# emolch/kiwi

Hardware: AMD Instinct MI355X
Metric: trial-source misfit evals/s (higher is better)
Workload: dtype f32

## Files before the change

kiwi_amd/csrc/kiwi_accum.hip:

```cpp
#include "kiwi_accum_api.hpp"

#if KIWI_ARITH == 0
#define KIWI_ARITH_NS exact
#elif KIWI_ARITH == 1
#define KIWI_ARITH_NS fused
#else
#error "KIWI_ARITH: 0 (exact) or 1 (fused)"
#endif

namespace kiwi {
namespace KIWI_ARITH_NS {

#include "kiwi_accum.inc"

#define KIWI_COMMON_ARGS a.G, a.span, a.pitch, a.recs, a.cent_ofs, a.isrc0, a.nrec, a.recv, a.syn, a.syn_stride

#if KIWI_FAMILY == 1
void launch_direct(const AccumArgs &a, dim3 grid)
{
    if (a.ng == 10) hipLaunchKernelGGL(accumulate_kernel<10>, grid, dim3(256), 0, a.stream, KIWI_COMMON_ARGS, a.synrow);
    else            hipLaunchKernelGGL(accumulate_kernel<8>, grid, dim3(256), 0, a.stream, KIWI_COMMON_ARGS, a.synrow);
}
#endif

// ... 22 lines not shown
    } else {
        if (T == 64) grouped_t<8, 64>(a, grid, ntiles, runs, pairsel, mate, mate4);
        else if (T == 128) grouped_t<8, 128>(a, grid, ntiles, runs, pairsel, mate, mate4);
        else grouped_t<8, 256>(a, grid, ntiles, runs, pairsel, mate, mate4);
    }
}
#endif

#if KIWI_FAMILY == 3
template <int NG, int NS, bool COMPACT, bool PLAN>
static void multi_t(const AccumArgs &a, dim3 grid, int ntiles, const int *mate, const int *wider)
{
    if (a.fuse) hipLaunchKernelGGL((accumulate_multi_kernel<NG, true, NS, COMPACT, PLAN>), grid, dim3(256), 0, a.stream, KIWI_COMMON_ARGS, ntiles, a.tab, a.coefs, a.fp,
                                   a.pairflag, mate, wider, a.plan, a.plan_ofs);
    else        hipLaunchKernelGGL((accumulate_multi_kernel<NG, false, NS, COMPACT, PLAN>), grid, dim3(256), 0, a.stream, KIWI_COMMON_ARGS, ntiles, a.tab, a.coefs, a.fp,
                                   a.pairflag, mate, wider, a.plan, a.plan_ofs);
}
template <int NG, int NS>
static void multi_c(const AccumArgs &a, dim3 grid, int ntiles, const int *mate, const int *wider)
{
    if (a.compact && a.plan) multi_t<NG, NS, true, true>(a, grid, ntiles, mate, wider);
    else if (a.compact) multi_t<NG, NS, true, false>(a, grid, ntiles, mate, wider);
    else multi_t<NG, NS, false, false>(a, grid, ntiles, mate, wider);
}
void launch_multi(const AccumArgs &a, dim3 grid, int NS, int ntiles, const int *mate, const int *wider)
{
    if (a.ng == 10) { if (NS == 4) multi_c<10, 4>(a, grid, ntiles, mate, wider); else multi_c<10, 2>(a, grid, ntiles, mate, wider); }
    else            { if (NS == 4) multi_c<8, 4>(a, grid, ntiles, mate, wider); else multi_c<8, 2>(a, grid, ntiles, mate, wider); }
}
void launch_multi_plan(const AccumArgs &a, int NS, int ngroups, const int *mate, const int *wider, PlanSrc *plan)
{
    const dim3 grid((unsigned)ngroups, (unsigned)((a.nrec + 63) / 64));
    if (NS == 4) hipLaunchKernelGGL(multi_plan_kernel<4>, grid, dim3(64), 0, a.stream, a.recs, a.cent_ofs, a.isrc0, a.nrec, a.recv, a.tab, a.pairflag, mate, wider,
                                    a.plan_ofs, (int4 *)plan, a.plan_regular, a.plan_count);
    else         hipLaunchKernelGGL(multi_plan_kernel<2>, grid, dim3(64), 0, a.stream, a.recs, a.cent_ofs, a.isrc0, a.nrec, a.recv, a.tab, a.pairflag, mate, wider,
                                    a.plan_ofs, (int4 *)plan, a.plan_regular, a.plan_count);
}
#endif

#if KIWI_FAMILY == 4
template <int NG, bool COMPACT>
static void cell_t(const AccumArgs &a, dim3 grid, int ntiles, bool per_wave)
{
#define KIWI_C(KERNEL) hipLaunchKernelGGL(KERNEL, grid, dim3(256), 0, a.stream, KIWI_COMMON_ARGS, ntiles, a.tab, a.coefs, a.fp, a.pairflag, a.synrow, \
                                          a.fam_ofs, a.fam_list)
    if (per_wave) { if (a.fuse) KIWI_C((accumulate_cellw_kernel<NG, true, COMPACT>)); else KIWI_C((accumulate_cellw_kernel<NG, false, COMPACT>)); }
    else          { if (a.fuse) KIWI_C((accumulate_cell_kernel<NG, 256, 2, 0, true, COMPACT>)); else KIWI_C((accumulate_cell_kernel<NG, 256, 2, 0, false, COMPACT>)); }
#undef KIWI_C
}
template <int NG>
static void cell_c(const AccumArgs &a, dim3 grid, int ntiles, bool per_wave)
{
    if (a.compact) cell_t<NG, true>(a, grid, ntiles, per_wave); else cell_t<NG, false>(a, grid, ntiles, per_wave);
}
void launch_cell(const AccumArgs &a, dim3 grid, int ntiles) { if (a.ng == 10) cell_c<10>(a, grid, ntiles, false); else cell_c<8>(a, grid, ntiles, false); }
void launch_cellw(const AccumArgs &a, dim3 grid, int ntiles) { if (a.ng == 10) cell_c<10>(a, grid, ntiles, true); else cell_c<8>(a, grid, ntiles, true); }
int cellw_range() { return kCellwRange; }
#endif

}
}
```

kiwi_amd/csrc/kiwi_accum.inc:

```


typedef float f4u __attribute__((ext_vector_type(4), aligned(4)));
typedef float f2u __attribute__((ext_vector_type(2), aligned(4)));

#if defined(KIWI_EXPLICIT_FMA)
#ifndef KIWI_CELLW_AHEAD
#define KIWI_CELLW_AHEAD 3
#endif
template <class V> __device__ __forceinline__ V kiwi_mad(V acc, float w, V v)
{
    V ws;
    for (int k = 0; k < (int)(sizeof(V) / sizeof(float)); k++) ws[k] = w;
    return __builtin_elementwise_fma(ws, v, acc);
}
template <class V> __device__ __forceinline__ V kiwi_madv(V acc, V w, V v) { return __builtin_elementwise_fma(w, v, acc); }
#else
template <class V> __device__ __forceinline__ V kiwi_mad(V acc, float w, V v) { return acc + w * v; }
template <class V> __device__ __forceinline__ V kiwi_madv(V acc, V w, V v) { return acc + w * v; }
#endif

typedef int v4i_t __attribute__((ext_vector_type(4)));
typedef int v2i_t __attribute__((ext_vector_type(2)));
__device__ __forceinline__ __amdgpu_buffer_rsrc_t gf_rsrc(const float *base)
{
// ... 788 lines not shown
        if constexpr (i < nH1) {
            t1[0] = t1[0] + c1 * s2a<i>(H); t1[0] = t1[0] + c2 * s2a<i>(L);
            t1[1] = t1[1] + c1 * s2b<i>(H); t1[1] = t1[1] + c2 * s2b<i>(L);
        } else if constexpr (i < nH1 + 2) {
            t2[0] = t2[0] + c1 * s2a<i>(H); t2[0] = t2[0] + c2 * s2a<i>(L);
            t2[1] = t2[1] + c1 * s2b<i>(H); t2[1] = t2[1] + c2 * s2b<i>(L);
        } else {
            dz[0] = dz[0] + c1 * s2a<i>(H); dz[0] = dz[0] + c2 * s2a<i>(L);
            dz[1] = dz[1] + c1 * s2b<i>(H); dz[1] = dz[1] + c2 * s2b<i>(L);
        }
        if constexpr (i == nH1 + 1) {
#pragma unroll
            for (int k = 0; k < 2; k++) {
                if (ROT) {
                    ar1[k] = ar1[k] + cl * t1[k] - sl * t2[k];
                    ar2[k] = ar2[k] + cl * t2[k] + sl * t1[k];
                } else {
                    ar1[k] = t1[k]; ar2[k] = t2[k];
                }
            }
        }
    });
}

template <int NG>
__device__ __forceinline__ typename Set2Sel<NG>::type make_set2(f2v &a0, f2v &a1, f2v &a2, f2v &a3, f2v &a4, f2v &a5, f2v &a6, f2v &a7, f2v &a8, f2v &a9,
                                                                f2v &b0, f2v &b1, f2v &b2, f2v &b3, f2v &b4, f2v &b5, f2v &b6, f2v &b7, f2v &b8, f2v &b9)
{
    if constexpr (NG == 10) return Set2_10{ a0, a1, a2, a3, a4, a5, a6, a7, a8, a9, b0, b1, b2, b3, b4, b5, b6, b7, b8, b9 };
    else return Set2_8{ a0, a1, a2, a3, a4, a5, a6, a7, b0, b1, b2, b3, b4, b5, b6, b7 };
}

#include "kiwi_apply_asm.inc"
#include "kiwi_apply_plan_asm.inc"
__device__ __forceinline__ int coef_warm(const float *p)
{
    int d;
    asm volatile("s_load_dword %0, %1, 0x0\n\ts_load_dword %0, %1, 0x40\n\ts_load_dword %0, %1, 0x80\n\ts_load_dword %0, %1, 0xc0\n\t"
                 "s_load_dword %0, %1, 0x100\n\ts_load_dword %0, %1, 0x140\n\ts_load_dword %0, %1, 0x180\n\ts_load_dword %0, %1, 0x1c0"
                 : "=&s"(d) : "s"(p) : "memory");
    return d;
}
#if KIWI_ARITH == 1
#define KIWI_APPLY_ASM(NGV, KV, RV) apply_group_asm_##NGV##_k##KV##_##RV##_fused
#define KIWI_APPLY_PLAN(NGV, KV, RV) apply_plan_asm_##NGV##_k##KV##_##RV##_fused
#else
#define KIWI_APPLY_ASM(NGV, KV, RV) apply_group_asm_##NGV##_k##KV##_##RV##_exact
#define KIWI_APPLY_PLAN(NGV, KV, RV) apply_plan_asm_##NGV##_k##KV##_##RV##_exact
#endif

template <int NG, int T, bool FUSE, bool RUNS, bool COMPACT >
__global__ __launch_bounds__(T) __attribute__((amdgpu_waves_per_eu(3))) void accumulate_grouped_kernel(
    const float *__restrict__ G, const int2 *__restrict__ span, int pitch,
    const GeoRec *__restrict__ recs, const int *__restrict__ cent_ofs, int isrc0, int nrec,
    const RecvDev *__restrict__ recv, float *__restrict__ syn, size_t syn_stride, int ntiles,
    const int *__restrict__ tab, const float *__restrict__ coefs, const int *__restrict__ run_first, FuseParams fp,
    const int *__restrict__ pairflag ,
    int pairsel ,
    const int *__restrict__ mate, const int *__restrict__ mate4 ,
    const int *__restrict__ synrow ,
    const int *__restrict__ fam_ofs, const int *__restrict__ fam_list )
{
    constexpr bool compact = COMPACT;
    constexpr int TILE = 4 * T;
    constexpr int LDS_TILE = TILE + kHalo;
    __shared__ __attribute__((aligned(16))) float tiles[NG][LDS_TILE];
    const int s = RUNS ? run_first[blockIdx.x] : (int)blockIdx.x;
    const int s_end = RUNS ? run_first[blockIdx.x + 1] : s + 1;
    const bool multi = RUNS && s_end - s > 1;
    const int tile = blockIdx.y % ntiles, r = blockIdx.y / ntiles;
    const RecvDev &rv = recv[r];
    if (!rv.enabled) return;
    if (tile * TILE >= rv.wlen) return;
    if (pairsel == 1 && cell_pair(rv, pairflag, s, nrec, r)) return;
    if (pairsel == 3 && (multi_taken_fwd<4>(rv, pairflag, mate4, s, nrec, r) || multi_taken_fwd<2>(rv, pairflag, mate, s, nrec, r))) return;
    if (synrow && !multi && synrow[s] != s) return;
    const int tid = threadIdx.x;
    const int lane = tid & 63;
    const int t_tile0 = rv.wbeg + tile * TILE;
    const int cb = cent_ofs[isrc0], c0 = cent_ofs[isrc0 + s], nc = cent_ofs[isrc0 + s + 1] - c0;
    const GeoRec *__restrict__ rc = recs + ((size_t)(c0 - cb) * nrec + (size_t)r * nc);
// ... 457 lines not shown
            for (int s = 0; s < NS; s++)
                if (only < 0 || only == s) one_finish<true>(v[i], tile0 + s * SET, LDS_TILE, comp(i), p, gw[s]);
        }
        if (i + DEPTH < N && (i + DEPTH < N - 1 || last_ok)) issue(i + DEPTH);
    }
    if (whalo) {
#pragma unroll
        for (int s = 0; s < NS; s++)
            if (only < 0 || only == s) halo_finish<true>(hact, hv, tile0 + s * SET, LDS_TILE, hig, hph, gw[s]);
    }
}


__device__ __forceinline__ int smax_u(int a, int b) { int r; asm("s_max_i32 %0, %1, %2" : "=s"(r) : "s"(a), "s"(b) : "scc"); return r; }
__device__ __forceinline__ int smin_u(int a, int b) { int r; asm("s_min_i32 %0, %1, %2" : "=s"(r) : "s"(a), "s"(b) : "scc"); return r; }

template <int NS>
__device__ __forceinline__ bool multi_taken(const RecvDev &rv, const int *__restrict__ pairflag, const int *__restrict__ mate,
                                            int s, int nrec, int r)
{
    if (!mate) return false;
    const int a = s - s % NS;
    if (!mate[a / NS] || !rv.need_h || !rv.has_d) return false;
    int f = 0;
#pragma unroll
    for (int i = 0; i < NS; i++) f |= pairflag[(size_t)(a + i) * nrec + r];
    return f == 0;
}

template <int NS>
__global__ __launch_bounds__(64) void multi_plan_kernel(const GeoRec *__restrict__ recs, const int *__restrict__ cent_ofs, int isrc0, int nrec,
    const RecvDev *__restrict__ recv, const int *__restrict__ off4, const int *__restrict__ pairflag, const int *__restrict__ mate,
    const int *__restrict__ mate_wider, const int *__restrict__ plan_ofs, int4 *__restrict__ plan,
    int regular_on , unsigned *__restrict__ count )
{
    constexpr int TILE = 1024 / NS, LDS_TILE = TILE + kHalo;
    const int k = (int)blockIdx.x, s0 = NS * k, r = (int)(blockIdx.y * 64 + threadIdx.x);
    if (r >= nrec) return;
    const RecvDev &rv = recv[r];
    if (!rv.enabled) return;
    if (!multi_taken<NS>(rv, pairflag, mate, s0, nrec, r)) return;
    if constexpr (NS == 2) { if (multi_taken<4>(rv, pairflag, mate_wider, s0, nrec, r)) return; }
    const int cb = cent_ofs[isrc0];
    const int nc = cent_ofs[isrc0 + s0 + 1] - cent_ofs[isrc0 + s0];
    const size_t pbeg = (size_t)plan_ofs[k], pend = (size_t)plan_ofs[k + 1];
    size_t pi = pbeg + (size_t)r;
    for (int c = 0; c < nc && pi < pend; pi += (size_t)nrec) {
        const GeoRec *h[NS];
        int smaxs[NS], smins[NS], npos = 0;
        bool shared = true, same_rows = true;
#pragma unroll
        for (int i = 0; i < NS; i++) {
            h[i] = recs + ((size_t)(cent_ofs[isrc0 + s0 + i] - cb) * nrec + (size_t)r * nc + c);
            smaxs[i] = h[i]->ishift + ((h[i]->pad >> 8) & 0xff);
            smins[i] = h[i]->ishift - ((h[i]->pad >> 16) & 0xff);
            npos = max(npos, TILE + (smaxs[i] - smins[i]) + 8);
            if (i > 0) {
                same_rows = same_rows && h[i]->row[0] == h[0]->row[0] && h[i]->row[1] == h[0]->row[1] && h[i]->row[2] == h[0]->row[2] && h[i]->row[3] == h[0]->row[3];
                shared = shared && smaxs[i] == smaxs[0];
            }
        }
        shared = shared && same_rows;
        if (same_rows && !shared) {
            int smax_c = smaxs[0], smin_c = smins[0];
#pragma unroll
            for (int i = 1; i < NS; i++) { smax_c = max(smax_c, smaxs[i]); smin_c = min(smin_c, smins[i]); }
            if (TILE + (smax_c - smin_c) + 8 <= LDS_TILE) {
                shared = true;
                npos = TILE + (smax_c - smin_c) + 8;
#pragma unroll
                for (int i = 0; i < NS; i++) smaxs[i] = smax_c;
            }
        }
        const int glen = h[0]->pad & 0xff;
        int4 *__restrict__ out = plan + pi * (kPlanStride / 16);
        unsigned nreg = 0;
#pragma unroll
        for (int i = 0; i < NS; i++) {
            const int4 o = *(const int4 *)(off4 + ((size_t)(cent_ofs[isrc0 + s0 + i] - cb) * nrec + (size_t)r * nc + c) * 4);
            const int e0 = smaxs[i] - h[i]->ishift;
            bool regular = regular_on != 0 && e0 >= 0 && e0 <= kPlanE0Mask;
            for (int j = 1; j < glen && c + j < nc; j++) regular = regular && h[i][j].ishift == h[i][j - 1].ishift + 1;
            nreg += regular ? 1u : 0u;
            const int head = (h[i]->flags & 0xffff) | (regular ? (e0 << kPlanE0Shift) | kPlanRegularBit : 0) | (glen << 16) | ((shared ? 1 : 0) << 23) | ((npos - TILE) << 24);
            out[4 * i + 0] = make_int4(h[i]->row[0], h[i]->row[1], h[i]->row[2], h[i]->row[3]);
            out[4 * i + 1] = o;
            out[4 * i + 2] = make_int4(__float_as_int(h[i]->w[0]), __float_as_int(h[i]->w[1]), __float_as_int(h[i]->w[2]), __float_as_int(h[i]->w[3]));
            out[4 * i + 3] = make_int4(smaxs[i], head, __float_as_int(h[i]->cl), __float_as_int(h[i]->sl));
        }
        if (count) { atomicAdd(count, (unsigned)NS); atomicAdd(count + 1, nreg); }
        if (glen < 1) break;
        c += glen;
    }
}

typedef const __attribute__((address_space(4))) v4i_t *plan_cptr;
template <int NS>
__device__ __forceinline__ int plan_warm(size_t p)
{
    int d;
    if constexpr (NS == 4)
        asm volatile("s_load_dword %0, %1, 0x0\n\ts_load_dword %0, %1, 0x40\n\ts_load_dword %0, %1, 0x80\n\ts_load_dword %0, %1, 0xc0" : "=&s"(d) : "s"(p) : "memory");
    else
        asm volatile("s_load_dword %0, %1, 0x0\n\ts_load_dword %0, %1, 0x40" : "=&s"(d) : "s"(p) : "memory");
    return d;
}

template <int NG, bool FUSE, int NS, bool COMPACT ,
          bool PLAN >
__global__ __launch_bounds__(256) __attribute__((amdgpu_waves_per_eu(3))) void accumulate_multi_kernel(
    const float *__restrict__ G, const int2 *__restrict__ span, int pitch,
    const GeoRec *__restrict__ recs, const int *__restrict__ cent_ofs, int isrc0, int nrec,
    const RecvDev *__restrict__ recv, float *__restrict__ syn, size_t syn_stride, int ntiles,
    const int *__restrict__ tab, const float *__restrict__ coefs, FuseParams fp, const int *__restrict__ pairflag, const int *__restrict__ mate,
    const int *__restrict__ mate_wider ,
    const PlanSrc *__restrict__ plan, const int *__restrict__ plan_ofs )
{
    constexpr bool compact = COMPACT;
    static_assert(NS == 2 || NS == 4, "sources per workgroup");
    static_assert(!PLAN || COMPACT, "plans hold compact descriptors");
    constexpr int TILE = 1024 / NS, LDS_TILE = TILE + kHalo, K = LDS_TILE / 64, WPS = 4 / NS;
    constexpr int SET = multi_set_stride<NG, NS>();
    __shared__ __attribute__((aligned(16))) float tiles[NS * SET];
// ... 94 lines not shown
            }
        }
        }
        const int glen = PLAN ? glen_p : (g[0].pad & 0xff);
        const int cend = c + glen;
        int smax = smaxs[0];
        if constexpr (PLAN) smax = plan4(64 * sh + 48).x;
        else {
#pragma unroll
            for (int i = 1; i < NS; i++) if (sh == i) smax = smaxs[i];
        }
        int flags = 0, ishv = 0, warm_ = 0, pwarm_ = 0;
        float gcl = 0.f, gsl = 0.f;
        const float *__restrict__ coef_grp = nullptr;
        auto shadow = [&]() {
            if constexpr (PLAN) {
#pragma unroll
                for (int i = 0; i < NS; i++) {
                    const v4i_t w = plan4(64 * i + 32);
                    g[i].w[0] = __int_as_float(w.x); g[i].w[1] = __int_as_float(w.y); g[i].w[2] = __int_as_float(w.z); g[i].w[3] = __int_as_float(w.w);
                }
                const v4i_t me = plan4(64 * sh + 48);
                flags = me.y & 0xffff; gcl = __int_as_float(me.z); gsl = __int_as_float(me.w);
                if (c + glen < nc) pwarm_ = plan_warm<NS>(pcur + (size_t)(unsigned)pstep);
            } else {
#pragma unroll
            for (int i = 0; i < NS; i++) { g[i].w[0] = REC_F(cur[i], 4); g[i].w[1] = REC_F(cur[i], 5); g[i].w[2] = REC_F(cur[i], 6); g[i].w[3] = REC_F(cur[i], 7); }
            int curme = cur[0];
#pragma unroll
            for (int i = 1; i < NS; i++) if (sh == i) curme = cur[i];
            flags = REC_I(curme, 18);
            gcl = REC_F(curme, 16); gsl = REC_F(curme, 17);
            }
            if (!(PLAN && (flags & kPlanRegularBit))) { if (lane < glen) ishv = rc[c + lane].ishift; }
            const size_t crow = (base_me + c) * kCoefLine;
            const unsigned clo = __builtin_amdgcn_readfirstlane((unsigned)crow), chi = __builtin_amdgcn_readfirstlane((unsigned)(crow >> 32));
            coef_grp = coefs + (((size_t)chi << 32) | clo);
            if constexpr (NG == 10) warm_ = coef_warm(coef_grp);
        };
        auto noshadow = []() {};
#define KIWI_MULTI_BUILD(DESC, I0, ONLY, NPOS, SHADOW) do { \
            const int jb_ = t_tile0 - smaxs[I0] - 1;       \
            const float *__restrict__ Gg = G + (size_t)g[I0].row[0] * (size_t)pitch; \
            const bool fast = (DESC).fast(jb_, LDS_TILE, pitch, lane, NG); \
            const bool hact = hq < 16 * NG && hph < (NPOS); \
            const bool whalo = __builtin_amdgcn_ballot_w64(hact) != 0ull; \
            if (fast) multi_build<NG, true, NS>(&tiles[0], wv, lane, tid, jb_, Gg, pitch, DESC, g, ONLY, hact, whalo, hig, hph, SHADOW); \
            else      multi_build<NG, false, NS>(&tiles[0], wv, lane, tid, jb_, Gg, pitch, DESC, g, ONLY, hact, whalo, hig, hph, SHADOW); } while (0)
        __builtin_amdgcn_s_setprio(1);
        if constexpr (PLAN) {
            if (shared) KIWI_MULTI_BUILD(dp, 0, -1, npos, shadow);
            else {
                KIWI_MULTI_BUILD(dp, 0, 0, npos, shadow);
#pragma unroll
                for (int i = 1; i < NS; i++) {
                    const v4i_t rw = plan4(64 * i), of = plan4(64 * i + 16);
                    smaxs[i] = plan4(64 * i + 48).x;
                    g[i].row[0] = rw.x;
                    const DescPlan di{ { 0, (rw.y - rw.x) * pitch, (rw.z - rw.x) * pitch, (rw.w - rw.x) * pitch }, { of.x, of.y, of.z, of.w }, pitch, hoff };
                    KIWI_MULTI_BUILD(di, i, i, npos, noshadow);
                }
            }
            asm volatile("" :: "s"(pwarm_));
            pcur += (size_t)(unsigned)pstep;
        } else {
        if (shared) KIWI_MULTI_BUILD((DescLanes{ ta, tb }), 0, -1, npos, shadow);
        else {
// ... 667 lines not shown
```

kiwi_amd/csrc/kiwi_accum_api.hpp:

```cpp
#pragma once
#include "kiwi_common.hpp"

namespace kiwi {

struct AccumArgs {
    hipStream_t stream;
    int ng;
    bool fuse;
    const float *G; const int2 *span; int pitch;
    const GeoRec *recs; const int *cent_ofs; int isrc0, nrec;
    const RecvDev *recv; float *syn; size_t syn_stride;
    const int *tab; const float *coefs; FuseParams fp;
    const int *pairflag, *synrow, *fam_ofs, *fam_list;
    int compact;
    const PlanSrc *plan = nullptr;
    const int *plan_ofs = nullptr;
    int plan_regular = 1;
    unsigned *plan_count = nullptr;
};

#define KIWI_ACCUM_LAUNCHERS                                                                                                      \
                                                                 \
    void launch_direct(const AccumArgs &a, dim3 grid);                                                                            \
                  \
    void launch_grouped(const AccumArgs &a, dim3 grid, int T, int ntiles, const int *runs, int pairsel, const int *mate,          \
                        const int *mate4);                                                                                        \
                                                     \
    void launch_multi(const AccumArgs &a, dim3 grid, int NS, int ntiles, const int *mate, const int *mate_wider);                \
                \
    void launch_multi_plan(const AccumArgs &a, int NS, int ngroups, const int *mate, const int *mate_wider, PlanSrc *plan);      \
        \
    void launch_cell(const AccumArgs &a, dim3 grid, int ntiles);                                                                  \
    void launch_cellw(const AccumArgs &a, dim3 grid, int ntiles);                                                                 \
                               \
    int cellw_range();

namespace exact { KIWI_ACCUM_LAUNCHERS }
namespace fused { KIWI_ACCUM_LAUNCHERS }
#undef KIWI_ACCUM_LAUNCHERS

}
```

kiwi_amd/csrc/kiwi_common.hpp:

```cpp
#pragma once
#include <hip/hip_runtime.h>
#include <type_traits>

namespace kiwi {

constexpr int kRowPad = 32;
constexpr int kTile = 1024;
constexpr int kMaxComp = 5;
constexpr int kHalo = 64;
constexpr int kMaxGroup = 64;

struct GeoRec {
    int   row[4];
    float w[4];
    int   ishift;
    float wfrac;
    float f[6];
    float cl, sl;
    int   flags;
    int   pad;
};
static_assert(sizeof(GeoRec) == 80, "GeoRec layout");

struct GfMeta {
// ... 36 lines not shown
    int ntrans_max;
    int fl_lo, fl_ns, refxofs;
    int untapered, rf0, rf1, vertical;
    int spankind;
};

struct FftPair {
    long long fft_ofs;
    long long spec_ofs;
    int ntrans;
    int specofs;
    int filtofs;
    int slot;
};
static_assert(sizeof(FftPair) == 32, "FftPair layout");

struct ShakeRec {
    int slot[3];
    int np;
    int untapered;
    int rec;
};

constexpr int kCoefLine = 20;
struct PlanSrc {
    int   row[4];
    int   o[4];
    float w[4];
    int   smax;
    int   head;
    float cl, sl;
};
static_assert(sizeof(PlanSrc) == 64, "PlanSrc layout");
constexpr int kPlanE0Shift = 4, kPlanE0Mask = 0x7f, kPlanRegularBit = 1 << 11;
constexpr int kPlanStride = 256;
template <int NG> __host__ __device__ constexpr int coef_wl(int a) { return 2 * a; }
template <int NG> __host__ __device__ constexpr int coef_wr(int a) { return 2 * a + 1; }

constexpr int kSpanInts = 8;
__device__ __forceinline__ void strip_span(const int *__restrict__ sp, int kind, int &lo, int &hi)
{
    if (kind == 3) { lo = sp[4]; hi = sp[5]; return; }
    if (kind == 0) { lo = sp[0]; hi = sp[1]; return; }
    if (kind == 1) { lo = sp[2]; hi = sp[3]; return; }
    lo = min(sp[0], sp[2]); hi = max(sp[1], sp[3]);
}

struct EvalParams {
    int bilinear, xus, zus;
    int nrec;
    int isrc0;
    int cellmode;
    int nogaps;
};

__device__ __forceinline__ bool cell_pair(const RecvDev &rv, const int *__restrict__ pairflag, int s, int nrec, int r)
{
    return rv.need_h && rv.has_d && !(pairflag[(size_t)s * nrec + r] & 3);
}

template <int NS>
__device__ __forceinline__ bool multi_taken_fwd(const RecvDev &rv, const int *__restrict__ pairflag, const int *__restrict__ mate,
                                                int s, int nrec, int r)
{
    if (!mate) return false;
    const int a = s - s % NS;
    if (!mate[a / NS] || !rv.need_h || !rv.has_d) return false;
// ... 36 lines not shown
```

kiwi_amd/csrc/kiwi_hip.hip:

```cpp
#include "../../include/kiwi_hip.h"
#include "kiwi_host.hpp"
#include "kiwi_host_eikonal.hpp"
#include "kiwi_host_lm.hpp"
#include "kiwi_geometry.hpp"
#include "kiwi_misfit.hpp"
#include "kiwi_accum_api.hpp"
#include "kiwi_fmm_device.hpp"

#include <hip/hip_runtime.h>
#include <hipfft/hipfft.h>
#include <algorithm>
#include <array>
#include <map>
#include <tuple>
#include <cstdio>
#include <cstdlib>
#include <cstring>
#include <string>
#include <vector>
#include <stdexcept>
#include <omp.h>
#include <chrono>
#include <condition_variable>
#include <deque>
// ... 141 lines not shown
    std::vector<float> norm_h;
    std::vector<float> reft_h;
    DevBuf<RecvDev> recv_d;
    DevBuf<CompDev> comps_d;
    DevBuf<float> reft_d, tw_d, norm_d;
    DevBuf<int> recfirst_d;
    int max_wlen = 0;

    int nsrc = 0;
    std::vector<int> cent_ofs;
    float max_risetime = 0.f;
    DevBuf<float> cent_d, moment_d, risetime_d;
    DevBuf<int> centofs_d;
    std::vector<int> src_status;
    bool any_failed = false;
    DevBuf<int> status_d;
    std::vector<int> same_as;
    bool any_same = false;
    DevBuf<int> synrow_d, famofs_d, famlist_d;
    int dedupe_enabled = 1;
    std::vector<unsigned long long> geo_hash;
    std::vector<kiwi_hip_ctx *> mates;
    int cpu_share = 1;
    std::vector<unsigned long long> struct_hash;
    std::vector<int> ngroups;
    std::vector<unsigned char> group_lens;
    std::vector<int> first_shift;
    std::vector<float> src_ends;
    DevBuf<int> mate_d, mate4_d;
    DevBuf<int> planofs_d;
    DevBuf<int4> plan_d;
    int multi_plan = 1;
    int multi_regular = 1;
    DevBuf<unsigned> plancount_d;
    int duo = 4;
    std::vector<char> single_group;
    DevBuf<int> runfirst_d;
    int share_runs = 1, max_run = 64;
    int fuse_enabled = 1;
    bool fuse_now = false;
    DevBuf<double> fusepart_d;

    DevBuf<float> misfit_d, global_d;
    DevBuf<GeoRec> recs_d;
    DevBuf<int> tab_d;
    DevBuf<int> off4_d;
    DevBuf<float> coef_d;
    DevBuf<int> pairflag_d;
    DevBuf<float> syn_d, proc_d;
    bool floating = false;
    int max_ns = 1;
    DevBuf<float> refx_d, vt_d, partial_d;
    DevBuf<int> fshift_d;
    int last_isrc0 = 0, last_nsrc = 0, last_chunk0 = 0, last_chunkn = 0;
    std::vector<char> evaluated;
    int last_proc_which = 0;
    int group_threads_env = 0;
    int group_threads = 128;
    int accum_mode = 0;
    int cell_mode = -1;
    int cell_wave = 1;
    int arith = KIWI_ARITH_EXACT;
    double points_per_centroid = 0.0;
    int keep_which = 0;
    int proc_chunk0 = 0, proc_chunkn = 0, proc_which_held = 0;
    size_t chunk_bytes_limit = (size_t)16 << 30;
// ... 919 lines not shown
                            HIPCHECK(hipMemcpyAsync(c->planofs_d.p, po, (n4 + n2 + 2) * sizeof(int), hipMemcpyHostToDevice, c->stream));
                            if (std::getenv("KIWI_HIP_POISON")) HIPCHECK(hipMemsetAsync(c->plan_d.p, 0x7f, (np + 1) * kPlanStride, c->stream));
                            planned = true;
                        }
                    }
                    HIPCHECK(hipEventRecord(c->mate_event, c->stream));
                }
            }
            const int ntiles_q = (c->max_wlen + 255) / 256;
            dim3 ggrid(gx, (unsigned)(ntiles * nrec));
            dim3 dgrid((unsigned)((nsrc + 1) / 2), (unsigned)(ntiles_p * nrec)), qgrid((unsigned)((nsrc + 3) / 4), (unsigned)(ntiles_q * nrec));
            dim3 cgrid((unsigned)nsrc, (unsigned)(ntiles_c * nrec));
            if (fuse) {
                const int nparts = cell ? std::max(ntiles * (T / 64), ntiles_c * (Tc / 64)) : (duo ? std::max({ ntiles * (T / 64), ntiles_p * 2, ntiles_q }) : ntiles * (T / 64));
                c->fusepart_d.ensure((size_t)nsrc * c->nmis * nparts, &c->dev_bytes);
                if (cell || duo) HIPCHECK(hipMemsetAsync(c->fusepart_d.p, 0, (size_t)nsrc * c->nmis * nparts * sizeof(double), c->stream));
                aa.fp = FuseParams{ c->reft_d.p, c->tw_d.p, c->moment_d.p, c->fusepart_d.p, c->method, c->syn_factor, c->nmis, nparts, isrc0 };
                fuse_nparts = nparts;
            }
            fuse_T = T; fuse_tile = 4 * T; fuse_ntiles = ntiles; fuse_all = cell || duo;
            aa.pairflag = (cell || duo) ? c->pairflag_d.p : (const int *)nullptr;
            if (cell) {
                static const bool cell_fused = [] { const char *e = std::getenv("KIWI_HIP_CELL_FUSED"); return !e || std::atoi(e) != 0; }();
                if (c->cell_wave) { if (fusedar && cell_fused) fused::launch_cellw(aa, cgrid, ntiles_c); else exact::launch_cellw(aa, cgrid, ntiles_c); }
                else exact::launch_cell(aa, cgrid, ntiles_c);
            }
            const int *m2p = any2 ? c->mate_d.p : (const int *)nullptr, *m4p = any4 ? c->mate4_d.p : (const int *)nullptr;
            AccumArgs aa4 = aa, aa2 = aa;
            if (planned) {
                const size_t n4 = (size_t)(nsrc + 3) / 4;
                aa4.plan = (const PlanSrc *)c->plan_d.p; aa4.plan_ofs = c->planofs_d.p;
                aa2.plan = (const PlanSrc *)(c->plan_d.p + plan_n4 * (kPlanStride / 16)); aa2.plan_ofs = c->planofs_d.p + n4 + 1;
                aa4.plan_regular = aa2.plan_regular = c->multi_regular;
                const bool count_plans = std::getenv("KIWI_HIP_DEBUG") != nullptr;
                if (count_plans) {
                    c->plancount_d.ensure(2, &c->dev_bytes);
                    HIPCHECK(hipMemsetAsync(c->plancount_d.p, 0, 2 * sizeof(unsigned), c->stream));
                    aa4.plan_count = aa2.plan_count = c->plancount_d.p;
                }
                if (any4) { if (fusedar) fused::launch_multi_plan(aa4, 4, (int)qgrid.x, m4p, nullptr, (PlanSrc *)aa4.plan); else exact::launch_multi_plan(aa4, 4, (int)qgrid.x, m4p, nullptr, (PlanSrc *)aa4.plan); }
                if (any2) { if (fusedar) fused::launch_multi_plan(aa2, 2, (int)dgrid.x, m2p, m4p, (PlanSrc *)aa2.plan); else exact::launch_multi_plan(aa2, 2, (int)dgrid.x, m2p, m4p, (PlanSrc *)aa2.plan); }
                if (count_plans) {
                    unsigned cnt[2] = { 0u, 0u };
                    HIPCHECK(hipMemcpyAsync(cnt, c->plancount_d.p, sizeof(cnt), hipMemcpyDeviceToHost, c->stream));
                    HIPCHECK(hipStreamSynchronize(c->stream));
                    std::fprintf(stderr, "[kiwi_hip] multi plans: %u of a (source, centroid group, receiver), %u regular\n", cnt[0], cnt[1]);
                }
            }
            if (any4) { if (fusedar) fused::launch_multi(aa4, qgrid, 4, ntiles_q, m4p, nullptr); else exact::launch_multi(aa4, qgrid, 4, ntiles_q, m4p, nullptr); }
            if (any2) { if (fusedar) fused::launch_multi(aa2, dgrid, 2, ntiles_p, m2p, m4p); else exact::launch_multi(aa2, dgrid, 2, ntiles_p, m2p, m4p); }
            const int pairsel = cell ? 1 : (duo ? 3 : 0);
            if (fusedar) fused::launch_grouped(aa, ggrid, T, ntiles, runs, pairsel, m2p, m4p);
            else         exact::launch_grouped(aa, ggrid, T, ntiles, runs, pairsel, m2p, m4p);
        }
    }
    record(c, 1, e2);
    if (c->any_untapered) {
        c->synspan_d.ensure((size_t)nsrc * c->nmis * 2, &c->dev_bytes);
        hipLaunchKernelGGL(synspan_kernel, dim3((unsigned)c->nmis, (unsigned)nsrc), dim3(256), 0, c->stream, c->syn_d.p, c->syn_stride, c->comps_d.p,
                           c->risetime_d.p + isrc0, c->gm.dt, c->nmis, spansrc, nrec, synrow, c->synspan_d.p);
    }
    if (c->untapered_fft) {
        const size_t np = (size_t)nsrc * c->nmis;
        c->ntr_d.ensure(np, &c->dev_bytes);
        pin_ensure(c->ntr_pin, c->ntr_pin_n, np);
        hipLaunchKernelGGL(fft_size_kernel, dim3((unsigned)((np + 255) / 256)), dim3(256), 0, c->stream, spansrc, c->comps_d.p, c->nmis,
                           nsrc, nrec, c->risetime_d.p + isrc0, c->gm.dt, c->ntr_d.p, (const int *)c->synspan_d.p);
        HIPCHECK(hipMemcpyAsync(c->ntr_pin, c->ntr_d.p, np * sizeof(int), hipMemcpyDeviceToHost, c->stream));
        HIPCHECK(hipEventRecord(c->size_event, c->stream));
    }
    if (c->fft_needed) layout_fft_chunk(c, isrc0, nsrc);
    {
        const bool spectral = (c->method == KIWI_AMPSPEC_L2NORM || c->method == KIWI_AMPSPEC_L1NORM);
        const int fl_method = c->method == KIWI_FLOATING_L2NORM ? KIWI_L2NORM : KIWI_L1NORM;
        const int td_method = spectral ? KIWI_L2NORM : (c->floating ? fl_method : c->method);
        const int fft_mode = !c->fft_needed ? 0 : (spectral ? 3 : 1);
        MisfitParams mp{ td_method, c->gm.dt, c->syn_factor, c->nmis, isrc0, proc_which == 3 ? 2 : proc_which, fft_mode, nsrc,
                         c->floating ? 1 : 0 };
        if (c->floating) {
// ... 176 lines not shown
        for (int k = 0; k < 8; k++) v[k] = __builtin_nontemporal_load(p + i + 256 * k);
#pragma unroll
        for (int k = 0; k < 8; k++) { x ^= v[k].x; y ^= v[k].y; z ^= v[k].z; w ^= v[k].w; }
    }
    for (; i < b; i += 256) { const read_u4 v = p[i]; x ^= v.x; y ^= v.y; z ^= v.z; w ^= v.w; }
    if ((x ^ y ^ z ^ w) == 0x9e3779b9u) sink[blockIdx.x] = x;
}

extern "C" {

int kiwi_hip_init(int device, kiwi_hip_ctx **out)
{
    kmp_set_blocktime(0);
    kiwi_hip_ctx *c = nullptr;
    try {
        int ndev = 0;
        hipError_t e = hipGetDeviceCount(&ndev);
        if (e != hipSuccess || ndev <= 0)
            return fail(nullptr, std::string("no HIP device available: ") + hipGetErrorString(e));
        if (device < 0 || device >= ndev) return fail(nullptr, "device index out of range");
        HIPCHECK(hipSetDevice(device));
        c = new kiwi_hip_ctx();
        c->device = device;
        HIPCHECK(hipStreamCreateWithFlags(&c->stream, hipStreamNonBlocking));
        if (const char *m = std::getenv("KIWI_HIP_GROUP_THREADS")) {
            const int v = std::atoi(m);
            if (v == 64 || v == 128 || v == 256) { c->group_threads = v; c->group_threads_env = 1; }
        }
        if (const char *m = std::getenv("KIWI_HIP_ACCUM")) c->accum_mode = (std::strcmp(m, "direct") == 0) ? 1 : 0;
        if (const char *m = std::getenv("KIWI_HIP_FUSE")) c->fuse_enabled = std::atoi(m);
        if (const char *m = std::getenv("KIWI_HIP_DUO")) { const int v = std::atoi(m); c->duo = v >= 4 ? 4 : (v >= 1 ? 2 : 0); }
        if (const char *m = std::getenv("KIWI_HIP_MULTI_PLAN")) c->multi_plan = std::atoi(m) ? 1 : 0;
        if (const char *m = std::getenv("KIWI_HIP_MULTI_REGULAR")) c->multi_regular = std::atoi(m) ? 1 : 0;
        if (const char *m = std::getenv("KIWI_HIP_CELL")) c->cell_mode = std::atoi(m) ? 1 : 0;
        if (const char *m = std::getenv("KIWI_HIP_DEDUPE")) c->dedupe_enabled = std::atoi(m);
        if (const char *m = std::getenv("KIWI_HIP_FUSED_FFT")) c->fused_fft = std::atoi(m) != 0;
        if (const char *m = std::getenv("KIWI_HIP_ARITH")) {
            if (std::strcmp(m, "fused") == 0 || std::strcmp(m, "fma") == 0) c->arith = KIWI_ARITH_FUSED;
            else if (std::strcmp(m, "exact") != 0) throw std::runtime_error("KIWI_HIP_ARITH: exact or fused");
        }
        if (const char *m = std::getenv("KIWI_HIP_CELL_WAVE")) c->cell_wave = std::atoi(m) ? 1 : 0;
        if (const char *m = std::getenv("KIWI_HIP_COMPACT")) c->compact = std::atoi(m) ? 1 : 0;
        if (const char *m = std::getenv("KIWI_HIP_CHUNK_MB")) {
            const long v = std::atol(m);
            if (v > 0) c->chunk_bytes_limit = (size_t)v << 20;
        }
        if (const char *m = std::getenv("KIWI_HIP_EIK_DEVICE")) c->eik_solver = std::atoi(m) ? 1 : 0;
        if (const char *m = std::getenv("KIWI_HIP_RUNS")) {
            const int v = std::atoi(m);
            c->share_runs = v != 0;
            if (v > 1) c->max_run = v;
        }
        *out = c;
        return 0;
    } catch (const std::exception &e) {
        delete c;
        return fail(nullptr, e.what());
    }
}

int kiwi_hip_init_multi(int ndev_wanted, kiwi_hip_ctx **out)
{
    if (!out) return fail(nullptr, "null argument");
    *out = nullptr;
    int ndev = 0;
    hipError_t e = hipGetDeviceCount(&ndev);
// ... 2456 lines not shown
```

profiles/kernel_resources.py:

```python
#!/usr/bin/env python3
import json
import os
import re
import subprocess
import sys

ROOT = os.path.dirname(os.path.dirname(os.path.abspath(__file__)))
CSRC = os.path.join(ROOT, "kiwi_amd", "csrc")
FAMILIES = {1: "direct", 2: "grouped", 3: "multi", 4: "cell"}


def demangle(names):
    out = subprocess.run(["c++filt"], input="\n".join(names), capture_output=True, text=True).stdout.split("\n")
    return [re.sub(r"\(.*", "", o).replace("void kiwi::", "").replace("void outer::", "outer::").replace("void bands::", "bands::").replace("void timescan::", "timescan::").replace("void linfit_timescan::", "linfit_timescan::").replace("void linfit::", "linfit::").replace("void linfit_candidates_timescan::", "linfit_candidates_timescan::").replace("void linfit_candidates_floating::", "linfit_candidates_floating::").replace("void spectral_candidates::", "spectral_candidates::") for o in out]


KEYS = (("sgpr", r"TotalSGPRs: (\d+)"), ("vgpr", r"\bVGPRs: (\d+)"), ("agpr", r"AGPRs: (\d+)"),
        ("scratch", r"ScratchSize \[bytes/lane\]: (\d+)"), ("occupancy", r"Occupancy \[waves/SIMD\]: (\d+)"),
        ("sgpr_spill", r"SGPRs Spill: (\d+)"), ("vgpr_spill", r"VGPRs Spill: (\d+)"), ("lds", r"LDS Size \[bytes/block\]: (\d+)"))


def collect_outer():
    r = subprocess.run(["make", "-s", "-C", CSRC, "asm-hip"], capture_output=True, text=True)
    rows, cur = [], None
    for line in (r.stderr + r.stdout).split("\n"):
        m = re.search(r"Function Name: (\S+)", line)
        if m:
            cur = None
            for prefix, fam in (("_ZN5outer", "outer"), ("_ZN5bands", "bands"), ("_ZN8timescan", "timescan"),
                                ("_ZN15linfit_timescan", "linfit_timescan"),
                                ("_ZN26linfit_candidates_timescan", "linfit_candidates_timescan"),
                                ("_ZN26linfit_candidates_floating", "linfit_candidates_floating"),
                                ("_ZN19spectral_candidates", "spectral_candidates")):
                if m.group(1).startswith(prefix):
                    cur = {"family": fam, "arith": "exact", "mangled": m.group(1)}
                    rows.append(cur)
            continue
        if cur is None:
            continue
        for key, pat in KEYS:
            m = re.search(pat, line)
            if m:
                cur[key] = int(m.group(1))
    return rows


def collect(only=None):
    rows = []
    for fam in ([] if only else FAMILIES):
        for ar in ("exact", "fused"):
            r = subprocess.run(["make", "-s", "-C", CSRC, "asm", "FAMILY=%d" % fam, "ARITH=%s" % ar], capture_output=True, text=True)
            txt = r.stderr + r.stdout
            cur = None
            for line in txt.split("\n"):
                m = re.search(r"Function Name: (\S+)", line)
                if m:
                    cur = {"family": FAMILIES[fam], "arith": ar, "mangled": m.group(1)}
                    rows.append(cur)
                    continue
                if cur is None:
                    continue
                for key, pat in (("sgpr", r"TotalSGPRs: (\d+)"), ("vgpr", r"\bVGPRs: (\d+)"), ("agpr", r"AGPRs: (\d+)"),
                                 ("scratch", r"ScratchSize \[bytes/lane\]: (\d+)"), ("occupancy", r"Occupancy \[waves/SIMD\]: (\d+)"),
                                 ("sgpr_spill", r"SGPRs Spill: (\d+)"), ("vgpr_spill", r"VGPRs Spill: (\d+)"),
                                 ("lds", r"LDS Size \[bytes/block\]: (\d+)")):
                    m = re.search(pat, line)
                    if m:
                        cur[key] = int(m.group(1))
    rows += [r for r in collect_outer() if not only or r["family"] == only]
    names = demangle([r["mangled"] for r in rows])
    for r, n in zip(rows, names):
        r["kernel"] = n
        del r["mangled"]
    return rows


def main():
    only = [a.split("=", 1)[1] for a in sys.argv[1:] if a.startswith("--only=")]
    rows = collect(only[0] if only else None)
    print("| kernel | contract | VGPR | AGPR | SGPR | VGPR spills | SGPR spills | scratch B/lane | LDS B | waves/SIMD |")
    print("|---|---|---|---|---|---|---|---|---|---|")
    for r in rows:
        print("| `%s` | %s | %d | %d | %d | %d | %d | %d | %d | %d |" % (r["kernel"], r["arith"], r.get("vgpr", -1), r.get("agpr", 0), r.get("sgpr", -1),
                                                                       r.get("vgpr_spill", 0), r.get("sgpr_spill", 0), r.get("scratch", 0),
                                                                       r.get("lds", 0), r.get("occupancy", -1)))
    if "--json" in sys.argv:
        json.dump(rows, open(sys.argv[sys.argv.index("--json") + 1], "w"), indent=1)


if __name__ == "__main__":
    main()
```

Measured before the change: 37490.

## Encode repeated-shift step patterns in multi plans to skip per-lane ishift loads

Extends the multi-source plan builder to detect groups whose time shifts advance by 0 or 1 per step (short groups up to length 5). It encodes the positions of the repeats as a bitmask in the plan header, so the apply kernel can rebuild the shifts from e0 plus the mask instead of loading per-lane ishift values. Apply now uses a new steps assembly include that handles the repeat mask. Adds an env toggle and a debug counter, and the profile script gains a code-size column. Risk: more header decoding in the hot apply path and larger generated code.

```diff
diff --git a/kiwi_amd/csrc/kiwi_accum.hip b/kiwi_amd/csrc/kiwi_accum.hip
--- a/kiwi_amd/csrc/kiwi_accum.hip
+++ b/kiwi_amd/csrc/kiwi_accum.hip
@@ -78,9 +78,9 @@
 {
     const dim3 grid((unsigned)ngroups, (unsigned)((a.nrec + 63) / 64));
     if (NS == 4) hipLaunchKernelGGL(multi_plan_kernel<4>, grid, dim3(64), 0, a.stream, a.recs, a.cent_ofs, a.isrc0, a.nrec, a.recv, a.tab, a.pairflag, mate, wider,
-                                    a.plan_ofs, (int4 *)plan, a.plan_regular, a.plan_count);
+                                    a.plan_ofs, (int4 *)plan, a.plan_regular, a.plan_repeat, a.plan_count);
     else         hipLaunchKernelGGL(multi_plan_kernel<2>, grid, dim3(64), 0, a.stream, a.recs, a.cent_ofs, a.isrc0, a.nrec, a.recv, a.tab, a.pairflag, mate, wider,
-                                    a.plan_ofs, (int4 *)plan, a.plan_regular, a.plan_count);
+                                    a.plan_ofs, (int4 *)plan, a.plan_regular, a.plan_repeat, a.plan_count);
 }
 #endif
 
diff --git a/kiwi_amd/csrc/kiwi_accum.inc b/kiwi_amd/csrc/kiwi_accum.inc
--- a/kiwi_amd/csrc/kiwi_accum.inc
+++ b/kiwi_amd/csrc/kiwi_accum.inc
@@ -844,7 +844,7 @@
 }
 
 #include "kiwi_apply_asm.inc"
-#include "kiwi_apply_plan_asm.inc"
+#include "kiwi_apply_steps_asm.inc"
 __device__ __forceinline__ int coef_warm(const float *p)
 {
     int d;
@@ -855,10 +855,10 @@
 }
 #if KIWI_ARITH == 1
 #define KIWI_APPLY_ASM(NGV, KV, RV) apply_group_asm_##NGV##_k##KV##_##RV##_fused
-#define KIWI_APPLY_PLAN(NGV, KV, RV) apply_plan_asm_##NGV##_k##KV##_##RV##_fused
+#define KIWI_APPLY_PLAN(NGV, KV, RV) apply_steps_asm_##NGV##_k##KV##_##RV##_fused
 #else
 #define KIWI_APPLY_ASM(NGV, KV, RV) apply_group_asm_##NGV##_k##KV##_##RV##_exact
-#define KIWI_APPLY_PLAN(NGV, KV, RV) apply_plan_asm_##NGV##_k##KV##_##RV##_exact
+#define KIWI_APPLY_PLAN(NGV, KV, RV) apply_steps_asm_##NGV##_k##KV##_##RV##_exact
 #endif
 
 template <int NG, int T, bool FUSE, bool RUNS, bool COMPACT >
@@ -1382,7 +1382,8 @@
 __global__ __launch_bounds__(64) void multi_plan_kernel(const GeoRec *__restrict__ recs, const int *__restrict__ cent_ofs, int isrc0, int nrec,
     const RecvDev *__restrict__ recv, const int *__restrict__ off4, const int *__restrict__ pairflag, const int *__restrict__ mate,
     const int *__restrict__ mate_wider, const int *__restrict__ plan_ofs, int4 *__restrict__ plan,
-    int regular_on , unsigned *__restrict__ count )
+    int regular_on , int repeat_on ,
+    unsigned *__restrict__ count )
 {
     constexpr int TILE = 1024 / NS, LDS_TILE = TILE + kHalo;
     const int k = (int)blockIdx.x, s0 = NS * k, r = (int)(blockIdx.y * 64 + threadIdx.x);
@@ -1424,21 +1425,31 @@
         }
         const int glen = h[0]->pad & 0xff;
         int4 *__restrict__ out = plan + pi * (kPlanStride / 16);
-        unsigned nreg = 0;
+        unsigned nreg = 0, nrep = 0;
 #pragma unroll
         for (int i = 0; i < NS; i++) {
             const int4 o = *(const int4 *)(off4 + ((size_t)(cent_ofs[isrc0 + s0 + i] - cb) * nrec + (size_t)r * nc + c) * 4);
             const int e0 = smaxs[i] - h[i]->ishift;
             bool regular = regular_on != 0 && e0 >= 0 && e0 <= kPlanE0Mask;
-            for (int j = 1; j < glen && c + j < nc; j++) regular = regular && h[i][j].ishift == h[i][j - 1].ishift + 1;
+            bool steps01 = regular && repeat_on != 0 && glen <= 5;
+            int repeats = 0;
+            for (int j = 1; j < glen && c + j < nc; j++) {
+                const int d = h[i][j].ishift - h[i][j - 1].ishift;
+                regular = regular && d == 1;
+                steps01 = steps01 && (d == 0 || d == 1);
+                if (d == 0 && j <= 4) repeats |= 1 << (j - 1);
+            }
+            if (regular || !steps01) repeats = 0;
             nreg += regular ? 1u : 0u;
-            const int head = (h[i]->flags & 0xffff) | (regular ? (e0 << kPlanE0Shift) | kPlanRegularBit : 0) | (glen << 16) | ((shared ? 1 : 0) << 23) | ((npos - TILE) << 24);
+            nrep += repeats ? 1u : 0u;
+            const int head = (h[i]->flags & 0xffff) | (regular || repeats ? (e0 << kPlanE0Shift) | (regular ? kPlanRegularBit : 0) | (repeats << kPlanRepeatShift) : 0)
+                             | (glen << 16) | ((shared ? 1 : 0) << 23) | ((npos - TILE) << 24);
             out[4 * i + 0] = make_int4(h[i]->row[0], h[i]->row[1], h[i]->row[2], h[i]->row[3]);
             out[4 * i + 1] = o;
             out[4 * i + 2] = make_int4(__float_as_int(h[i]->w[0]), __float_as_int(h[i]->w[1]), __float_as_int(h[i]->w[2]), __float_as_int(h[i]->w[3]));
             out[4 * i + 3] = make_int4(smaxs[i], head, __float_as_int(h[i]->cl), __float_as_int(h[i]->sl));
         }
-        if (count) { atomicAdd(count, (unsigned)NS); atomicAdd(count + 1, nreg); }
+        if (count) { atomicAdd(count, (unsigned)NS); atomicAdd(count + 1, nreg); atomicAdd(count + 2, nrep); }
         if (glen < 1) break;
         c += glen;
     }
@@ -1599,7 +1610,7 @@
             flags = REC_I(curme, 18);
             gcl = REC_F(curme, 16); gsl = REC_F(curme, 17);
             }
-            if (!(PLAN && (flags & kPlanRegularBit))) { if (lane < glen) ishv = rc[c + lane].ishift; }
+            if (!(PLAN && (flags & (kPlanRegularBit | kPlanRepeatMask)))) { if (lane < glen) ishv = rc[c + lane].ishift; }
             const size_t crow = (base_me + c) * kCoefLine;
             const unsigned clo = __builtin_amdgcn_readfirstlane((unsigned)crow), chi = __builtin_amdgcn_readfirstlane((unsigned)(crow >> 32));
             coef_grp = coefs + (((size_t)chi << 32) | clo);
diff --git a/kiwi_amd/csrc/kiwi_accum_api.hpp b/kiwi_amd/csrc/kiwi_accum_api.hpp
--- a/kiwi_amd/csrc/kiwi_accum_api.hpp
+++ b/kiwi_amd/csrc/kiwi_accum_api.hpp
@@ -16,6 +16,7 @@
     const PlanSrc *plan = nullptr;
     const int *plan_ofs = nullptr;
     int plan_regular = 1;
+    int plan_repeat = 1;
     unsigned *plan_count = nullptr;
 };
 
diff --git a/kiwi_amd/csrc/kiwi_common.hpp b/kiwi_amd/csrc/kiwi_common.hpp
--- a/kiwi_amd/csrc/kiwi_common.hpp
+++ b/kiwi_amd/csrc/kiwi_common.hpp
@@ -92,7 +92,7 @@
     float cl, sl;
 };
 static_assert(sizeof(PlanSrc) == 64, "PlanSrc layout");
-constexpr int kPlanE0Shift = 4, kPlanE0Mask = 0x7f, kPlanRegularBit = 1 << 11;
+constexpr int kPlanE0Shift = 4, kPlanE0Mask = 0x7f, kPlanRegularBit = 1 << 11, kPlanRepeatShift = 12, kPlanRepeatMask = 0xf << kPlanRepeatShift;
 constexpr int kPlanStride = 256;
 template <int NG> __host__ __device__ constexpr int coef_wl(int a) { return 2 * a; }
 template <int NG> __host__ __device__ constexpr int coef_wr(int a) { return 2 * a + 1; }
diff --git a/kiwi_amd/csrc/kiwi_hip.hip b/kiwi_amd/csrc/kiwi_hip.hip
--- a/kiwi_amd/csrc/kiwi_hip.hip
+++ b/kiwi_amd/csrc/kiwi_hip.hip
@@ -197,6 +197,7 @@
     DevBuf<int4> plan_d;
     int multi_plan = 1;
     int multi_regular = 1;
+    int multi_repeat = 1;
     DevBuf<unsigned> plancount_d;
     int duo = 4;
     std::vector<char> single_group;
@@ -1182,19 +1183,21 @@
                 aa4.plan = (const PlanSrc *)c->plan_d.p; aa4.plan_ofs = c->planofs_d.p;
                 aa2.plan = (const PlanSrc *)(c->plan_d.p + plan_n4 * (kPlanStride / 16)); aa2.plan_ofs = c->planofs_d.p + n4 + 1;
                 aa4.plan_regular = aa2.plan_regular = c->multi_regular;
+                aa4.plan_repeat = aa2.plan_repeat = c->multi_repeat;
                 const bool count_plans = std::getenv("KIWI_HIP_DEBUG") != nullptr;
                 if (count_plans) {
-                    c->plancount_d.ensure(2, &c->dev_bytes);
-                    HIPCHECK(hipMemsetAsync(c->plancount_d.p, 0, 2 * sizeof(unsigned), c->stream));
+                    c->plancount_d.ensure(3, &c->dev_bytes);
+                    HIPCHECK(hipMemsetAsync(c->plancount_d.p, 0, 3 * sizeof(unsigned), c->stream));
                     aa4.plan_count = aa2.plan_count = c->plancount_d.p;
                 }
                 if (any4) { if (fusedar) fused::launch_multi_plan(aa4, 4, (int)qgrid.x, m4p, nullptr, (PlanSrc *)aa4.plan); else exact::launch_multi_plan(aa4, 4, (int)qgrid.x, m4p, nullptr, (PlanSrc *)aa4.plan); }
                 if (any2) { if (fusedar) fused::launch_multi_plan(aa2, 2, (int)dgrid.x, m2p, m4p, (PlanSrc *)aa2.plan); else exact::launch_multi_plan(aa2, 2, (int)dgrid.x, m2p, m4p, (PlanSrc *)aa2.plan); }
                 if (count_plans) {
-                    unsigned cnt[2] = { 0u, 0u };
+                    unsigned cnt[3] = { 0u, 0u, 0u };
                     HIPCHECK(hipMemcpyAsync(cnt, c->plancount_d.p, sizeof(cnt), hipMemcpyDeviceToHost, c->stream));
                     HIPCHECK(hipStreamSynchronize(c->stream));
                     std::fprintf(stderr, "[kiwi_hip] multi plans: %u of a (source, centroid group, receiver), %u regular\n", cnt[0], cnt[1]);
+                    std::fprintf(stderr, "[kiwi_hip] multi plans with named repeats: %u\n", cnt[2]);
                 }
             }
             if (any4) { if (fusedar) fused::launch_multi(aa4, qgrid, 4, ntiles_q, m4p, nullptr); else exact::launch_multi(aa4, qgrid, 4, ntiles_q, m4p, nullptr); }
@@ -1437,6 +1440,7 @@
         if (const char *m = std::getenv("KIWI_HIP_DUO")) { const int v = std::atoi(m); c->duo = v >= 4 ? 4 : (v >= 1 ? 2 : 0); }
         if (const char *m = std::getenv("KIWI_HIP_MULTI_PLAN")) c->multi_plan = std::atoi(m) ? 1 : 0;
         if (const char *m = std::getenv("KIWI_HIP_MULTI_REGULAR")) c->multi_regular = std::atoi(m) ? 1 : 0;
+        if (const char *m = std::getenv("KIWI_HIP_MULTI_REPEAT")) c->multi_repeat = std::atoi(m) ? 1 : 0;
         if (const char *m = std::getenv("KIWI_HIP_CELL")) c->cell_mode = std::atoi(m) ? 1 : 0;
         if (const char *m = std::getenv("KIWI_HIP_DEDUPE")) c->dedupe_enabled = std::atoi(m);
         if (const char *m = std::getenv("KIWI_HIP_FUSED_FFT")) c->fused_fft = std::atoi(m) != 0;
diff --git a/profiles/kernel_resources.py b/profiles/kernel_resources.py
--- a/profiles/kernel_resources.py
+++ b/profiles/kernel_resources.py
@@ -45,10 +45,19 @@
     return rows
 
 
-def collect(only=None):
+def text_sizes(fam, ar):
+    subprocess.run(["make", "-s", "-C", CSRC, "co", "FAMILY=%d" % fam, "ARITH=%s" % ar], capture_output=True, text=True, check=True)
+    readelf = os.path.join(os.environ.get("ROCM_PATH", "/opt/rocm"), "llvm", "bin", "llvm-readelf")
+    out = subprocess.run([readelf, "-s", "-W", os.path.join(CSRC, "build", "accum_%d_%s.co" % (fam, ar))], capture_output=True, text=True, check=True).stdout
+    return {f[7]: int(f[2]) for f in (line.split() for line in out.split("\n")) if len(f) == 8 and f[3] == "FUNC"}
+
+
+def collect(only=None, text=False):
     rows = []
-    for fam in ([] if only else FAMILIES):
+    accum = [f for f, n in FAMILIES.items() if n == only] if only in FAMILIES.values() else ([] if only else FAMILIES)
+    for fam in accum:
         for ar in ("exact", "fused"):
+            sizes = text_sizes(fam, ar) if text else {}
             r = subprocess.run(["make", "-s", "-C", CSRC, "asm", "FAMILY=%d" % fam, "ARITH=%s" % ar], capture_output=True, text=True)
             txt = r.stderr + r.stdout
             cur = None
@@ -56,6 +65,8 @@
                 m = re.search(r"Function Name: (\S+)", line)
                 if m:
                     cur = {"family": FAMILIES[fam], "arith": ar, "mangled": m.group(1)}
+                    if m.group(1) in sizes:
+                        cur["text"] = sizes[m.group(1)]
                     rows.append(cur)
                     continue
                 if cur is None:
@@ -67,7 +78,8 @@
                     m = re.search(pat, line)
                     if m:
                         cur[key] = int(m.group(1))
-    rows += [r for r in collect_outer() if not only or r["family"] == only]
+    if only not in FAMILIES.values():
+        rows += [r for r in collect_outer() if not only or r["family"] == only]
     names = demangle([r["mangled"] for r in rows])
     for r, n in zip(rows, names):
         r["kernel"] = n
@@ -77,13 +89,14 @@
 
 def main():
     only = [a.split("=", 1)[1] for a in sys.argv[1:] if a.startswith("--only=")]
-    rows = collect(only[0] if only else None)
-    print("| kernel | contract | VGPR | AGPR | SGPR | VGPR spills | SGPR spills | scratch B/lane | LDS B | waves/SIMD |")
-    print("|---|---|---|---|---|---|---|---|---|---|")
+    text = "--text" in sys.argv
+    rows = collect(only[0] if only else None, text)
+    print("| kernel | contract | VGPR | AGPR | SGPR | VGPR spills | SGPR spills | scratch B/lane | LDS B | waves/SIMD |%s" % (" text B |" if text else ""))
+    print("|---|---|---|---|---|---|---|---|---|---|%s" % ("---|" if text else ""))
     for r in rows:
-        print("| `%s` | %s | %d | %d | %d | %d | %d | %d | %d | %d |" % (r["kernel"], r["arith"], r.get("vgpr", -1), r.get("agpr", 0), r.get("sgpr", -1),
-                                                                       r.get("vgpr_spill", 0), r.get("sgpr_spill", 0), r.get("scratch", 0),
-                                                                       r.get("lds", 0), r.get("occupancy", -1)))
+        print("| `%s` | %s | %d | %d | %d | %d | %d | %d | %d | %d |%s" % (r["kernel"], r["arith"], r.get("vgpr", -1), r.get("agpr", 0), r.get("sgpr", -1),
+                                                                         r.get("vgpr_spill", 0), r.get("sgpr_spill", 0), r.get("scratch", 0),
+                                                                         r.get("lds", 0), r.get("occupancy", -1), (" %d |" % r.get("text", -1)) if text else ""))
     if "--json" in sys.argv:
         json.dump(rows, open(sys.argv[sys.argv.index("--json") + 1], "w"), indent=1)
 
```

New measurement: 39530, median of 6. 5.5% higher.
